# d8ahazard/AudioLab

Measured on AMD Instinct MI355X. Metric: stems*realtime-factor (44.1kHz stereo), higher is better.
Workload: dtype bf16; 1 GPU; MDX-Net UVR 4-stem (4x TFC-TDF U-Net L=11 g=48 dim_f=3072 dim_t=256 n_fft=6144), 300 s 44.1 kHz stereo in total, margin chunker, windows/launch=52; stems=4

## Files before the change

audiolab_amd/csrc/tdfnet.hip:

```cpp
#include "mma.h"
#include <alsep_gfx950_asm.h>

#include <map>
#include <type_traits>

namespace {

constexpr int kThreads = 256;

template <typename T> struct Vec16;
template <> struct Vec16<float> { static constexpr int N = 4; };
template <> struct Vec16<bf16_t> { static constexpr int N = 8; };
__device__ __forceinline__ void store_vec(float* p, const float* y) { *reinterpret_cast<float4*>(p) = make_float4(y[0], y[1], y[2], y[3]); }
__device__ __forceinline__ void store_vec(bf16_t* p, const float* y) {
    bf16x8 q;
#pragma unroll
    for (int e = 0; e < 8; ++e) q[e] = (bf16_t)y[e];
    *reinterpret_cast<bf16x8*>(p) = q;
}
__device__ __forceinline__ void load_vec(const float* p, float* x) {
    const float4 q = *reinterpret_cast<const float4*>(p);
    x[0] = q.x; x[1] = q.y; x[2] = q.z; x[3] = q.w;
}
__device__ __forceinline__ void load_vec(const bf16_t* p, float* x) {
// ... 566 lines not shown
        if (i < Cf::WINST) glds16(wsrc_next + ((size_t)i * 64 + lane) * 8, wdst_next + (size_t)i * 64 * 8);
    };

    constexpr int ST = 4 * (Cf::NPAIR + Cf::NB % 2);
    f32x4 acc[NY][3][4];
    if (nstage > 0) {
        issue_patch(0);
        weights_prep(0);
#pragma unroll
        for (int j = 0; j < 6; ++j) weights_one(j);
    }
    for (int s = 0; s < nstage; ++s) {
        const int ny = s % NY, ps = s / NY, q = ps % nq;
        const bool last = s + 1 >= nstage;
        const bool after_epilogue = ny == 0 && q == 0 && s > 0;
        if (after_epilogue) wait_vmcnt<ST>();
        else wait_vmcnt<0>();
        barrier_nodrain();
        if (!last) weights_prep(s + 1);
        {
            const bf16_t* wts = wring + (size_t)(s & 1) * Cf::WGROUPS * 8;
#pragma unroll
            for (int yy = 0; yy < NY; ++yy) {
                if (yy == ny) {
                    if (q == 0) {
#pragma unroll
                        for (int mi = 0; mi < 3; ++mi)
#pragma unroll
                            for (int ni = 0; ni < 4; ++ni) acc[yy][mi][ni] = f32x4{0.f, 0.f, 0.f, 0.f};
                    }
#pragma unroll 2
                    for (int st = 0; st < Cf::NS; ++st) {
                        const int ko = koff_of(st);
                        bf16x8 xf[4], wf[3];
#pragma unroll
                        for (int ni = 0; ni < 4; ++ni) xf[ni] = lds_frag<bf16_t>(patch + pbase[ni] + ko);
#pragma unroll
                        for (int mi = 0; mi < 3; ++mi)
                            wf[mi] = lds_frag<bf16_t>(wts + ((mi * 16 + l15) * Cf::WGRP + ((4 * st + lq) ^ wswz)) * 8);
#pragma unroll
                        for (int mi = 0; mi < 3; ++mi)
#pragma unroll
                            for (int ni = 0; ni < 4; ++ni) mma_step(acc[yy][mi][ni], wf[mi], xf[ni]);
                        if (st < 6 && !last) weights_one(st);
                    }
                }
            }
        }
        if (ny == NY - 1) {
            barrier_nodrain();
            if (!last) issue_patch(ps + 1);
            if (q == nq - 1) {
                int t0, f0; int64_t b;
                tile_coords(ps / nq, t0, f0, b);
                bf16_t* yb = Y + ((b * Th + t0 + wave) * (int64_t)Fw + f0) * Cout;
#pragma unroll
                for (int ni = 0; ni < 4; ++ni) {
                    bf16_t* yp = yb + (int64_t)(ni * 16 + l15) * Cout;
#pragma unroll
                    for (int j = 0; j < Cf::NPAIR; ++j) {
                        const int co = j * 32 + lq * 8;
                        float y[8];
#pragma unroll
                        for (int h = 0; h < 2; ++h) {
                            const int bb = 2 * j + h;
                            const f32x4 scv = *reinterpret_cast<const f32x4*>(ss + co + 4 * h);
                            const f32x4 shv = *reinterpret_cast<const f32x4*>(ss + NY * Cf::BN + co + 4 * h);
#pragma unroll
                            for (int r = 0; r < 4; ++r) y[4 * h + r] = fmaxf(fmaf(acc[bb / 3][bb % 3][ni][r], scv[r], shv[r]), 0.f);
                        }
                        store8(yp + co, y);
                    }
                    if constexpr (Cf::NB % 2 == 1) {
                        constexpr int bb = Cf::NB - 1;
                        const int co = bb * 16 + lq * 4;
                        const f32x4 scv = *reinterpret_cast<const f32x4*>(ss + co);
                        const f32x4 shv = *reinterpret_cast<const f32x4*>(ss + NY * Cf::BN + co);
                        float y[4];
#pragma unroll
                        for (int r = 0; r < 4; ++r) y[r] = fmaxf(fmaf(acc[bb / 3][bb % 3][ni][r], scv[r], shv[r]), 0.f);
                        store4(yp + co, y);
                    }
                }
            }
        }
    }
}

struct ConvMq {
    static constexpr int NY = 2, TW = 64, TH = 8, KC = 32, CG = 4, NS = 9, PW = TW + 2, PH = TH + 2;
    static constexpr int PARTS = 2, KS = 5;
    static constexpr int WG = 4 * KS, ROWS = 96, NB = 6, NPAIR = 3;
    static constexpr int PGROUPS = PH * PW * CG, PINST = (PGROUPS + 63) / 64, PJ = (PINST + 7) / 8;
    static constexpr int WGROUPS = ROWS * WG, WINST = WGROUPS / 64, WJ = (WINST + 7) / 8;
    static constexpr int PBUF = PINST * 64;
    static constexpr size_t ring_bytes = 16 * (size_t)(2 * PBUF + 2 * WGROUPS);
    static constexpr size_t lds_bytes = ring_bytes + 2 * ROWS * sizeof(float) + 1024;
    static_assert(lds_bytes <= 160 * 1024, "ConvMq: LDS budget");
    __host__ __device__ static constexpr int ksteps_of_part(int pt) { return pt == 0 ? KS : NS - KS; }
    __host__ __device__ static constexpr int wswz(int row) { return (4 - ((row >> 2) & 3)) & 3; }
    __host__ __device__ static constexpr int pswz(int pix) { return ((pix >> 2) & 1) << 1; }
};

template <int TAP, int STL>
__device__ __forceinline__ void mq_issue_reads(bf16x8 (&xf)[4], bf16x8 (&wf)[6], const bf16_t* patch, const int (&pk)[9], const bf16_t* wl) {
    typedef ConvMq Cf;
    const bf16_t* pl = patch + pk[TAP];
    lds_read_async_b128<0 * 16 * Cf::KC * 2>(xf[0], pl);
    lds_read_async_b128<1 * 16 * Cf::KC * 2>(xf[1], pl);
    lds_read_async_b128<2 * 16 * Cf::KC * 2>(xf[2], pl);
    lds_read_async_b128<3 * 16 * Cf::KC * 2>(xf[3], pl);
    lds_read_async_b128<(0 * 16 * Cf::WG * 8 + STL * 32) * 2>(wf[0], wl);
    lds_read_async_b128<(1 * 16 * Cf::WG * 8 + STL * 32) * 2>(wf[1], wl);
    lds_read_async_b128<(2 * 16 * Cf::WG * 8 + STL * 32) * 2>(wf[2], wl);
    lds_read_async_b128<(3 * 16 * Cf::WG * 8 + STL * 32) * 2>(wf[3], wl);
    lds_read_async_b128<(4 * 16 * Cf::WG * 8 + STL * 32) * 2>(wf[4], wl);
    lds_read_async_b128<(5 * 16 * Cf::WG * 8 + STL * 32) * 2>(wf[5], wl);
}
__device__ __forceinline__ void mq_mma(f32x4 (&acc)[6][4], const bf16x8 (&wf)[6], const bf16x8 (&xf)[4]) {
#pragma unroll
    for (int b = 0; b < 6; ++b)
#pragma unroll
        for (int ni = 0; ni < 4; ++ni) mma_step(acc[b][ni], wf[b], xf[ni]);
}
template <int PT, int STL, typename Dma>
__device__ __forceinline__ void mq_steps(f32x4 (&acc)[6][4], bf16x8 (&xa)[4], bf16x8 (&wa)[6], bf16x8 (&xb)[4], bf16x8 (&wb)[6],
                                         const bf16_t* patch, const int (&pk)[9], const bf16_t* wl, Dma dma) {
    constexpr int N = ConvMq::ksteps_of_part(PT), T0 = PT * ConvMq::KS;
    if constexpr (STL < N) {
        if constexpr (STL == 0) mq_issue_reads<T0, 0>(xa, wa, patch, pk, wl);
        lds_wait_n<0>();
        if constexpr (STL + 1 < N) mq_issue_reads<T0 + STL + 1, STL + 1>(xb, wb, patch, pk, wl);
        mq_mma(acc, wa, xa);
        dma(STL);
        sched_fence();
        if constexpr (STL + 1 < N) {
            lds_wait_n<0>();
            if constexpr (STL + 2 < N) mq_issue_reads<T0 + STL + 2, STL + 2>(xa, wa, patch, pk, wl);
            mq_mma(acc, wb, xb);
            dma(STL + 1);
            sched_fence();
            mq_steps<PT, STL + 2>(acc, xa, wa, xb, wb, patch, pk, wl, dma);
        }
    }
}

__global__ void __launch_bounds__(kBigThreads, 2)
conv3x3_bf16_mq_kernel(const bf16_t* __restrict__ X, bf16_t* __restrict__ Y, const bf16_t* __restrict__ Wp, const float* __restrict__ scale,
                       const float* __restrict__ shift, const bf16_t* __restrict__ zero_page, int Th, int Fw, int Cin, int Cout, int tiles_t,
                       int tiles_f, int ntiles) {
    typedef ConvMq Cf;
    bf16_t* const patch0 = reinterpret_cast<bf16_t*>(alsep_smem);
    bf16_t* const wring = patch0 + (size_t)2 * Cf::PBUF * 8;
    float* ss = reinterpret_cast<float*>(alsep_smem + Cf::ring_bytes);
    bf16_t* const scratch = reinterpret_cast<bf16_t*>(alsep_smem + Cf::lds_bytes - 1024);
    const int tid = threadIdx.x, lane = tid & 63, wave = tid >> 6;
    const int l15 = lane & 15, lq = lane >> 4;
    const int nq = Cin / Cf::KC;
    for (int i = tid; i < Cf::ROWS; i += kBigThreads) {
        ss[i] = scale[i];
        ss[Cf::ROWS + i] = shift[i];
    }
    __syncthreads();

    int pk[9];
#pragma unroll
// ... 1638 lines not shown
            for (int ni = 0; ni < P::NI; ++ni) acc[mt][ni] = f32x4{0.f, 0.f, 0.f, 0.f};
        bf16x8 xf[2][P::NI];
        static_for<P::NI>([&](auto nic) {
            constexpr int ni = decltype(nic)::value;
            lds_read_async_b128<ni * 2 * P::XREG>(xf[0][ni], xs + bk[0] / sizeof(bf16_t));
        });
        static_for<P::KS>([&](auto ksc) {
            constexpr int ks = decltype(ksc)::value, b = ks & 1;
            if constexpr (ks + 1 < P::KS) {
                static_for<P::NI>([&](auto nic) {
                    constexpr int ni = decltype(nic)::value;
                    lds_read_async_b128<ni * 2 * P::XREG>(xf[1 - b][ni], xs + bk[ks + 1] / sizeof(bf16_t));
                });
                lds_wait_n<P::NI>();
            } else {
                lds_wait_n<0>();
                if (P::C % 32 != 0) {
#pragma unroll
                    for (int ni = 0; ni < P::NI; ++ni) xf[b][ni] = klast_ok ? xf[b][ni] : bf16x8{};
                }
            }
#pragma unroll
            for (int mt = 0; mt < P::MT; ++mt)
#pragma unroll
                for (int ni = 0; ni < P::NI; ++ni) mma_step(acc[mt][ni], wf[mt][ks], xf[b][ni]);
        });
        bf16_t* sl = reinterpret_cast<bf16_t*>(sring + (size_t)(i % P::NSS) * P::s_bytes + ebase);
        const float* bnl = bn + 4 * lq;
        auto eoff = [&](int mt) {
            int t = 2 * mt + erot;
            t = t >= P::NG ? t - P::NG : t;
            return t * 8;
        };
        bf16x8 ev[2][P::NI];
        f32x4 scv[2], shv[2];
        auto eread = [&](auto mtc) {
            constexpr int mt = decltype(mtc)::value, eb = mt & 1;
            const bf16_t* p = sl + eoff(mt);
            static_for<P::NI>([&](auto nic) {
                constexpr int ni = decltype(nic)::value;
                lds_read_async_b128<ni * 32 * P::NG * 16>(ev[eb][ni], p);
            });
            lds_read_async_f32x4<0>(scv[eb], bnl + mt * 16);
            lds_read_async_f32x4<P::C2 * 4>(shv[eb], bnl + mt * 16);
        };
        eread(std::integral_constant<int, 0>{});
        static_for<P::MT>([&](auto mtc) {
            constexpr int mt = decltype(mtc)::value, b = mt & 1;
            if constexpr (mt + 1 < P::MT) {
                eread(std::integral_constant<int, mt + 1>{});
                lds_wait_n<P::NI + 2>();
            } else {
                lds_wait_n<0>();
            }
            bf16_t* p = sl + eoff(mt) + (lq & 1) * 4;
            static_for<P::NI>([&](auto nic) {
                constexpr int ni = decltype(nic)::value;
                const bf16x4 sk = (lq & 1) ? __builtin_shufflevector(ev[b][ni], ev[b][ni], 4, 5, 6, 7)
                                           : __builtin_shufflevector(ev[b][ni], ev[b][ni], 0, 1, 2, 3);
                bf16x4 q;
#pragma unroll
                for (int r = 0; r < 4; ++r) q[r] = (bf16_t)(fmaxf(fmaf(acc[mt][ni][r], scv[b][r], shv[b][r]), 0.f) * (float)sk[r]);
                lds_write_async_b64(p + ni * 32 * P::NG * 8, q);
            });
        });
    }
    barrier_nodrain();
    copy_out(nmy - 1);
}

#ifndef ALSEP_F16_TU
#include "tdfnet_f32s.h"
#endif

struct DevBuf {
    void* p = nullptr;
    size_t bytes = 0;
};

struct ConvLayer {
    DevBuf w, scale, shift;
    DevBuf w_big;
    DevBuf w_mq;
    int cin = 0, cout = 0;
    bool dma_path = false;
    int split = 0;
    unsigned* range_flag = nullptr;
};
struct GemmLayer {
    DevBuf w, bias, scale, shift;
    int M = 0, K = 0, Kp = 0, Mp = 0;
    bool has_bias = false;
    bool split = false;
    unsigned* range_flag = nullptr;
    bool dma_path = false;
    DevBuf wfrag;
    DevBuf wwide;
};
struct Block {
    std::vector<ConvLayer> tfc;
    std::vector<GemmLayer> tdf;
};

}

struct alsep_net {
    alsep_ctx* ctx = nullptr;
    alsep_net_config cfg{};
    int n = 0;
    bool split = false;
    DevBuf range_flag;
    std::vector<DevBuf> owned;
    DevBuf first_w, first_scale, first_shift, final_w, final_b, zero_page;
    std::vector<Block> enc, dec;
    Block bott;
    std::vector<GemmLayer> ds, us;
};

namespace {

typedef std::map<std::string, std::vector<float>> TensorMap;

template <typename T> T host_cast(float v);
template <> float host_cast<float>(float v) { return v; }
template <> bf16_t host_cast<bf16_t>(float v) { return (bf16_t)v; }

int upload(alsep_net* net, const void* src, size_t bytes, DevBuf* out) {
    void* d = nullptr;
    if (hipMalloc(&d, bytes ? bytes : 16) != hipSuccess) return alsep_fail(net->ctx, ALSEP_ERR_NOMEM, "hipMalloc(%zu) failed", bytes);
    out->p = d;
    out->bytes = bytes;
    net->owned.push_back(*out);
    if (bytes) ALSEP_HIP(net->ctx, hipMemcpy(d, src, bytes, hipMemcpyHostToDevice));
    return ALSEP_OK;
}

const std::vector<float>* find(const TensorMap& tm, const std::string& name, int64_t numel, alsep_ctx* ctx, bool required = true) {
    auto it = tm.find(name);
    if (it == tm.end()) {
        if (required) alsep_fail(ctx, ALSEP_ERR_ARG, "missing tensor '%s'", name.c_str());
        return nullptr;
    }
    if ((int64_t)it->second.size() != numel) {
        alsep_fail(ctx, ALSEP_ERR_ARG, "tensor '%s' has %zu elements, expected %lld", name.c_str(), it->second.size(), (long long)numel);
        return nullptr;
    }
    return &it->second;
}

template <typename T> struct ConvSel;
template <> struct ConvSel<bf16_t> { static constexpr int KC = 48, BN = 48; };
template <> struct ConvSel<float> { static constexpr int KC = 16, BN = 48; };
template <typename T> struct ConvSel16;
template <> struct ConvSel16<bf16_t> { static constexpr int KC = 16, BN = 16; };
template <> struct ConvSel16<float> { static constexpr int KC = 16, BN = 16; };

template <typename T> bool conv_uses_main(int cin, int cout) {
    return cin % ConvSel<T>::KC == 0 && cout % ConvSel<T>::BN == 0;
}

template <typename T, int KC, int BN>
std::vector<T> pack_conv3x3(const std::vector<float>& w, int cin, int cout) {
    typedef ConvCfg<T, KC, BN, 64> Cf;
    const int nq = cin / KC, nn = cout / BN;
    std::vector<T> out((size_t)nn * nq * BN * Cf::KP, host_cast<T>(0.f));
    for (int j = 0; j < nn; ++j)
        for (int q = 0; q < nq; ++q)
            for (int r = 0; r < BN; ++r)
                for (int grp = 0; grp < Cf::NG; ++grp)
                    for (int e = 0; e < Cf::G; ++e) {
                        const int tap = grp / Cf::CG, cg = grp % Cf::CG;
                        const int ci = q * KC + cg * Cf::G + e, co = j * BN + r;
                        const float v = w[(((size_t)co * cin + ci) * 3 + tap / 3) * 3 + tap % 3];
                        out[(((size_t)j * nq + q) * BN + r) * Cf::KP + grp * Cf::G + e] = host_cast<T>(v);
                    }
    return out;
}

std::vector<bf16_t> pack_conv3x3_dma(const std::vector<float>& w, int cin, int cout) {
    typedef ConvB16<64> Cf;
    const int nq = cin / Cf::KC, nn = cout / Cf::BN;
    std::vector<bf16_t> out((size_t)nn * nq * Cf::WGROUPS * 8, host_cast<bf16_t>(0.f));
    for (int j = 0; j < nn; ++j)
        for (int q = 0; q < nq; ++q)
            for (int r = 0; r < Cf::BN; ++r)
                for (int grp = 0; grp < Cf::NG; ++grp)
                    for (int e = 0; e < 8; ++e) {
                        const int tap = grp / Cf::CG, cg = grp % Cf::CG;
                        const int ci = q * Cf::KC + cg * 8 + e, co = j * Cf::BN + r;
                        const float v = w[(((size_t)co * cin + ci) * 3 + tap / 3) * 3 + tap % 3];
                        const int pg = grp ^ ((r >> 1) & 7);
                        out[((((size_t)j * nq + q) * Cf::BN + r) * Cf::WG + pg) * 8 + e] = host_cast<bf16_t>(v);
                    }
    return out;
}

template <int NY>
std::vector<bf16_t> pack_conv3x3_big(const std::vector<float>& w, int cin) {
    const int cout = 48 * NY;
    std::vector<float> wp(w.size());
    const size_t row = (size_t)cin * 9;
    for (int R = 0; R < cout; ++R) std::copy(w.begin() + ConvBig<NY>::channel_of_row(R) * row, w.begin() + (ConvBig<NY>::channel_of_row(R) + 1) * row, wp.begin() + R * row);
    return pack_conv3x3_dma(wp, cin, cout);
}

std::vector<bf16_t> pack_conv3x3_mq(const std::vector<float>& w, int cin) {
    typedef ConvMq Cf;
    const int nq = cin / Cf::KC;
    std::vector<bf16_t> out((size_t)nq * Cf::PARTS * Cf::WGROUPS * 8, host_cast<bf16_t>(0.f));
    for (int q = 0; q < nq; ++q)
        for (int pt = 0; pt < Cf::PARTS; ++pt)
            for (int R = 0; R < Cf::ROWS; ++R)
                for (int stl = 0; stl < Cf::ksteps_of_part(pt); ++stl)
                    for (int lq = 0; lq < 4; ++lq) {
                        const int tap = pt * Cf::KS + stl, co = ConvBig<2>::channel_of_row(R);
                        const size_t dst = ((((size_t)q * Cf::PARTS + pt) * Cf::ROWS + R) * Cf::WG + 4 * stl + (lq ^ Cf::wswz(R))) * 8;
                        for (int e = 0; e < 8; ++e) {
                            const int ci = q * Cf::KC + lq * 8 + e;
                            out[dst + e] = host_cast<bf16_t>(w[(((size_t)co * cin + ci) * 3 + tap / 3) * 3 + tap % 3]);
                        }
                    }
    return out;
}

template <typename T> constexpr bool is_bf16() { return false; }
template <> constexpr bool is_bf16<bf16_t>() { return true; }

template <typename T>
int make_conv(alsep_net* net, const TensorMap& tm, const std::string& p, int c, ConvLayer* L) {
    auto w = find(tm, p + ".weight", (int64_t)c * c * 9, net->ctx);
    auto sc = find(tm, p + ".scale", c, net->ctx);
    auto sh = find(tm, p + ".shift", c, net->ctx);
    if (!w || !sc || !sh) return ALSEP_ERR_ARG;
    L->cin = L->cout = c;
    int rc;
#ifndef ALSEP_F16_TU
    if (!is_bf16<T>() && net->split && (c % 48 == 0 || c % 16 == 0)) {
        L->split = c % 48 == 0 ? 24 : 16;
        L->range_flag = (unsigned*)net->range_flag.p;
        const std::vector<hs_t> pk = L->split == 24 ? pack_conv3x3_split<24, 48>(*w, c, c) : pack_conv3x3_split<16, 16>(*w, c, c);
        rc = upload(net, pk.data(), pk.size() * sizeof(hs_t), &L->w);
    } else
#endif
    if (is_bf16<T>() && c % 48 == 0) {
        L->dma_path = true;
        auto pk = pack_conv3x3_dma(*w, c, c);
        rc = upload(net, pk.data(), pk.size() * sizeof(bf16_t), &L->w);
        if (!rc && c == 48) {
            auto p0 = pack_conv3x3_big<1>(*w, c);
            rc = upload(net, p0.data(), p0.size() * sizeof(bf16_t), &L->w_big);
        }
        if (!rc && c == 96) {
            auto pq = pack_conv3x3_mq(*w, c);
            rc = upload(net, pq.data(), pq.size() * sizeof(bf16_t), &L->w_mq);
        }
        if (!rc && c == 144) {
            auto pb = pack_conv3x3_big<3>(*w, c);
            rc = upload(net, pb.data(), pb.size() * sizeof(bf16_t), &L->w_big);
        }
    } else if (conv_uses_main<T>(c, c)) {
        auto pk = pack_conv3x3<T, ConvSel<T>::KC, ConvSel<T>::BN>(*w, c, c);
        rc = upload(net, pk.data(), pk.size() * sizeof(T), &L->w);
    } else {
        auto pk = pack_conv3x3<T, ConvSel16<T>::KC, ConvSel16<T>::BN>(*w, c, c);
        rc = upload(net, pk.data(), pk.size() * sizeof(T), &L->w);
    }
    if (rc) return rc;
    if ((rc = upload(net, sc->data(), c * sizeof(float), &L->scale))) return rc;
    return upload(net, sh->data(), c * sizeof(float), &L->shift);
}

template <typename T>
int make_gemm_weights(alsep_net* net, const std::vector<float>& wmk, int M, int K, GemmLayer* L) {
    typedef GemmCfg<T> Gc;
    L->M = M; L->K = K;
#ifndef ALSEP_F16_TU
    if (!is_bf16<T>() && net->split) {
        L->split = true;
        L->range_flag = (unsigned*)net->range_flag.p;
        const std::vector<hs_t> pk = pack_gemm_split(wmk, M, K, &L->Mp, &L->Kp);
        return upload(net, pk.data(), pk.size() * sizeof(hs_t), &L->w);
    }
#endif
    L->Mp = (int)ceil_div64(M, Gc::BR) * Gc::BR;
    L->Kp = (int)ceil_div64(K, Gc::BK) * Gc::BK;
    std::vector<T> pk((size_t)L->Mp * L->Kp, host_cast<T>(0.f));
    for (int m = 0; m < M; ++m)
        for (int k = 0; k < K; ++k) pk[(size_t)m * L->Kp + k] = host_cast<T>(wmk[(size_t)m * K + k]);
    return upload(net, pk.data(), pk.size() * sizeof(T), &L->w);
}

int make_tdf_dma_weights(alsep_net* net, const std::vector<float>& wmk, int M, int K, GemmLayer* L) {
    typedef TdfB16 Tc;
    L->M = M; L->K = K;
    L->Mp = (int)ceil_div64(M, Tc::BM) * Tc::BM;
    L->Kp = (int)ceil_div64(K, Tc::BK) * Tc::BK;
    L->dma_path = true;
    std::vector<bf16_t> pk((size_t)L->Mp * L->Kp, host_cast<bf16_t>(0.f));
    for (int m = 0; m < M; ++m)
        for (int kt = 0; kt < L->Kp / Tc::BK; ++kt)
            for (int g = 0; g < 8; ++g) {
                const int ks = g >> 2, lq = g & 3, pg = g ^ ((m >> 1) & 7);
                for (int e = 0; e < 8; ++e) {
                    const int k = kt * Tc::BK + ks * 32 + (e < 4 ? 4 * lq + e : 16 + 4 * lq + (e - 4));
                    if (k < K) pk[(size_t)m * L->Kp + kt * Tc::BK + pg * 8 + e] = host_cast<bf16_t>(wmk[(size_t)m * K + k]);
                }
            }
    return upload(net, pk.data(), pk.size() * sizeof(bf16_t), &L->w);
}

int make_tdf_wide_weights(alsep_net* net, const std::vector<float>& wmk, int M, int K, GemmLayer* L) {
    const int KT = (int)ceil_div64(K, 64);
    std::vector<bf16_t> pk((size_t)(M / 48) * KT * 6 * 512, host_cast<bf16_t>(0.f));
    for (int rb = 0; rb < M / 48; ++rb)
        for (int kt = 0; kt < KT; ++kt)
            for (int ks = 0; ks < 2; ++ks)
                for (int mi = 0; mi < 3; ++mi)
                    for (int l = 0; l < 64; ++l)
                        for (int e = 0; e < 8; ++e) {
                            const int lq = l >> 4, m = rb * 48 + mi * 16 + (l & 15);
                            const int k = kt * 64 + ks * 32 + (e < 4 ? 4 * lq + e : 16 + 4 * lq + (e - 4));
                            if (k < K)
                                pk[((((size_t)rb * KT + kt) * 2 + ks) * 3 + mi) * 512 + l * 8 + e] =
                                    host_cast<bf16_t>(wmk[(size_t)m * K + k]);
                        }
    return upload(net, pk.data(), pk.size() * sizeof(bf16_t), &L->wwide);
}

int make_frag_weights(alsep_net* net, const std::vector<float>& wmk, int M, int K, DevBuf* out) {
    const int MT = (M + 15) / 16, KS = (K + 31) / 32;
    std::vector<bf16_t> pk((size_t)MT * KS * 64 * 8, host_cast<bf16_t>(0.f));
    for (int mt = 0; mt < MT; ++mt)
        for (int ks = 0; ks < KS; ++ks)
            for (int l = 0; l < 64; ++l)
                for (int e = 0; e < 8; ++e) {
                    const int m = mt * 16 + (l & 15), k = ks * 32 + (l >> 4) * 8 + e;
                    if (m < M && k < K) pk[(((size_t)mt * KS + ks) * 64 + l) * 8 + e] = host_cast<bf16_t>(wmk[(size_t)m * K + k]);
                }
    return upload(net, pk.data(), pk.size() * sizeof(bf16_t), out);
}

template <typename T>
// ... 125 lines not shown
    return v;
}

template <int TW>
int launch_conv_dma(alsep_ctx* ctx, const ConvLayer& L, const bf16_t* X, bf16_t* Y, const bf16_t* zero_page, int64_t B,
                    int Th, int Fw) {
    typedef ConvB16<TW> Cf;
    const int tiles_t = (int)ceil_div64(Th, Cf::TH), tiles_f = (int)ceil_div64(Fw, TW);
    const int64_t ntiles = B * tiles_t * tiles_f;
    if (ntiles > 0x7fffffff) return alsep_fail(ctx, ALSEP_ERR_ARG, "conv3x3: too many tiles");
    ALSEP_HIP(ctx, hipFuncSetAttribute((const void*)conv3x3_bf16_kernel<TW>, hipFuncAttributeMaxDynamicSharedMemorySize,
                                       (int)Cf::lds_bytes));
    ProfScope prof(ctx, TW == 64 ? ALSEP_PROF_CONV3X3 : ALSEP_PROF_CONV3X3_SMALL);
    prof.work(18.0 * (double)L.cin * L.cout * B * Th * Fw, (double)sizeof(*X) * B * Th * Fw * (L.cin + L.cout));
    const int nyc = L.cout / Cf::BN;
    const int ny_fastest = conv_ny_fastest() && ntiles % 8 == 0 && nyc > 1 && ntiles * nyc <= 0x7fffffff;
    hipLaunchKernelGGL((conv3x3_bf16_kernel<TW>), ny_fastest ? dim3((unsigned)(ntiles * nyc)) : dim3((unsigned)ntiles, nyc),
                       dim3(kThreads), Cf::lds_bytes,
                       ctx->stream, X, Y, (const bf16_t*)L.w.p, (const float*)L.scale.p, (const float*)L.shift.p, zero_page,
                       Th, Fw, L.cin, L.cout, tiles_t, tiles_f, (int)ntiles,  0,  0, ny_fastest);
    note_launch(ctx, TW == 64 ? "conv3x3_bf16_kernel<64>" : "conv3x3_bf16_kernel<small>");
    ALSEP_LAUNCH_CHECK(ctx, "conv3x3_bf16_kernel");
    return ALSEP_OK;
}

template <int NQ, int RING_ = 3, int OCC = 1, int TW_ = 64>
int launch_conv_regw(alsep_ctx* ctx, const ConvLayer& L, const bf16_t* X, bf16_t* Y, const bf16_t* zero_page, int64_t B,
                     int Th, int Fw) {
    typedef ConvRW<NQ, RING_, TW_> Cf;
    const int tiles_t = Th / Cf::TH, tiles_f = Fw / Cf::TW;
    const int64_t ntiles = B * tiles_t * tiles_f;
    if (ntiles > 0x7fffffff) return alsep_fail(ctx, ALSEP_ERR_ARG, "conv3x3: too many tiles");
    ALSEP_HIP(ctx, hipFuncSetAttribute((const void*)conv3x3_bf16_regw_kernel<NQ, RING_, OCC, TW_>,
                                       hipFuncAttributeMaxDynamicSharedMemorySize, (int)Cf::lds_bytes));
    const int ny = L.cout / Cf::BN;
    int gx = OCC * 256 / ny;
    if (gx > ntiles) gx = (int)ntiles;
    ProfScope prof(ctx, ALSEP_PROF_CONV3X3_REGW);
    prof.work(18.0 * (double)L.cin * L.cout * B * Th * Fw, (double)sizeof(*X) * B * Th * Fw * (L.cin + L.cout));
    hipLaunchKernelGGL((conv3x3_bf16_regw_kernel<NQ, RING_, OCC, TW_>), dim3((unsigned)gx, ny), dim3(kThreads), Cf::lds_bytes, ctx->stream, X, Y,
                       (const bf16_t*)L.w.p, (const float*)L.scale.p, (const float*)L.shift.p, zero_page, Th, Fw, L.cin,
                       L.cout, tiles_t, tiles_f, (int)ntiles);
    ALSEP_LAUNCH_CHECK(ctx, "conv3x3_bf16_regw_kernel");
    return ALSEP_OK;
}

template <typename Cf, typename Kern>
int launch_conv_persist(alsep_ctx* ctx, Kern kern, const ConvLayer& L, const DevBuf& wimg, int prof_class, const char* name, const bf16_t* X,
                        bf16_t* Y, const bf16_t* zero_page, int64_t B, int Th, int Fw) {
    const int tiles_t = Th / Cf::TH, tiles_f = Fw / Cf::TW;
    const int64_t ntiles = B * tiles_t * tiles_f;
    if (ntiles > 0x7fffffff) return alsep_fail(ctx, ALSEP_ERR_ARG, "conv3x3: too many tiles");
    ALSEP_HIP(ctx, hipFuncSetAttribute((const void*)kern, hipFuncAttributeMaxDynamicSharedMemorySize, (int)Cf::lds_bytes));
    const int gx = ntiles < 256 ? (int)ntiles : 256;
    ProfScope prof(ctx, prof_class);
    prof.work(18.0 * (double)L.cin * L.cout * B * Th * Fw, (double)sizeof(*X) * B * Th * Fw * (L.cin + L.cout));
    hipLaunchKernelGGL(kern, dim3((unsigned)gx), dim3(kBigThreads), Cf::lds_bytes, ctx->stream, X, Y, (const bf16_t*)wimg.p,
                       (const float*)L.scale.p, (const float*)L.shift.p, zero_page, Th, Fw, L.cin, L.cout, tiles_t, tiles_f, (int)ntiles);
    ALSEP_LAUNCH_CHECK(ctx, name);
    return ALSEP_OK;
}

int launch_conv_big3(alsep_ctx* ctx, const ConvLayer& L, const bf16_t* X, bf16_t* Y, const bf16_t* zero_page, int64_t B, int Th, int Fw) {
    if (!L.w_big.p) return alsep_fail(ctx, ALSEP_ERR_STATE, "conv3x3: no big-tile weight image for this layer");
    if (int rc = launch_conv_persist<ConvBig<3>>(ctx, conv3x3_bf16_big_kernel<3>, L, L.w_big, ALSEP_PROF_CONV3X3_BIG3, "conv3x3_bf16_big_kernel",
                                                 X, Y, zero_page, B, Th, Fw))
        return rc;
    note_launch(ctx, "conv3x3_bf16_big_kernel<3>");
    return ALSEP_OK;
}

int launch_conv_mq(alsep_ctx* ctx, const ConvLayer& L, const bf16_t* X, bf16_t* Y, const bf16_t* zero_page, int64_t B, int Th, int Fw) {
    if (!L.w_mq.p || L.cout != ConvMq::ROWS || L.cin % ConvMq::KC) return alsep_fail(ctx, ALSEP_ERR_STATE, "conv3x3: no mq weight image for this layer");
    return launch_conv_persist<ConvMq>(ctx, conv3x3_bf16_mq_kernel, L, L.w_mq, ALSEP_PROF_CONV3X3_BIG, "conv3x3_bf16_mq_kernel", X, Y, zero_page,
                                       B, Th, Fw);
}

int launch_conv_m0(alsep_ctx* ctx, const ConvLayer& L, const bf16_t* X, bf16_t* Y, const bf16_t* zero_page, int64_t B, int Th, int Fw) {
    if (!L.w_big.p || L.cout != ConvM0::ROWS || L.cin != ConvM0::KC) return alsep_fail(ctx, ALSEP_ERR_STATE, "conv3x3: no m0 weight image for this layer");
    return launch_conv_persist<ConvM0>(ctx, conv3x3_bf16_m0_kernel, L, L.w_big, ALSEP_PROF_CONV3X3_REGW, "conv3x3_bf16_m0_kernel", X, Y, zero_page,
                                       B, Th, Fw);
}

int conv_m0_enabled() {
    static const int v = env_int("ALSEP_CONV_M0", 1);
    return v;
}
int conv_regw_enabled() {
    static const int v = env_int("ALSEP_CONV_REGW", 1);
    return v;
}
int conv_big_enabled() {
    static const int v = env_int("ALSEP_CONV_BIG", 1);
    return v;
}
int conv_mq_enabled() {
    static const int v = env_int("ALSEP_CONV_MQ", 1);
    return v;
}
int conv_big3_enabled() {
    static const int v = env_int("ALSEP_CONV_BIG3", 1);
    return v;
}

int run_conv_dma(alsep_ctx* ctx, const ConvLayer& L, const bf16_t* X, bf16_t* Y, const bf16_t* zp, int64_t B, int Th, int Fw) {
    if (conv_m0_enabled() && L.cin == 48 && L.cout == 48 && Th % 8 == 0 && Fw % 48 == 0 &&
        (conv_m0_enabled() >= 2 || B * (Th / 8) * (Fw / 48) >= 256))
        return launch_conv_m0(ctx, L, X, Y, zp, B, Th, Fw);
    if (conv_regw_enabled() && Th % 4 == 0 && Fw % 64 == 0 && L.cin == L.cout) {
        if (L.cin == 48 && conv_regw_enabled() == 3) return launch_conv_regw<1>(ctx, L, X, Y, zp, B, Th, Fw);
        if (L.cin == 48) return launch_conv_regw<1, 3, 2, 32>(ctx, L, X, Y, zp, B, Th, Fw);
        if (L.cin == 96 && conv_regw_enabled() >= 2) return launch_conv_regw<2>(ctx, L, X, Y, zp, B, Th, Fw);
    }
    if (conv_big_enabled() && Th % 8 == 0 && Fw % 64 == 0 && L.cin == L.cout &&
        (conv_big_enabled() >= 2 || B * (Th / 8) * (Fw / 64) >= 96)) {
        if (L.cout == 96 && conv_mq_enabled()) return launch_conv_mq(ctx, L, X, Y, zp, B, Th, Fw);
        if (L.cout == 144 && conv_big3_enabled()) return launch_conv_big3(ctx, L, X, Y, zp, B, Th, Fw);
    }
    if (Fw >= 64 && Fw % 64 == 0) return launch_conv_dma<64>(ctx, L, X, Y, zp, B, Th, Fw);
    if (Fw >= 32) return launch_conv_dma<32>(ctx, L, X, Y, zp, B, Th, Fw);
    return launch_conv_dma<16>(ctx, L, X, Y, zp, B, Th, Fw);
}
int run_conv_dma(alsep_ctx* ctx, const ConvLayer&, const float*, float*, const float*, int64_t, int, int) {
    return alsep_fail(ctx, ALSEP_ERR_STATE, "LDS-DMA conv path is bf16 only");
}

#ifndef ALSEP_F16_TU
template <int KC, int BN, int TW>
int launch_conv_split(alsep_ctx* ctx, const ConvLayer& L, const float* X, float* Y, int64_t B, int Th, int Fw) {
    typedef ConvSCfg<KC, BN, TW> Cf;
    const int tiles_t = (int)ceil_div64(Th, Cf::TH), tiles_f = (int)ceil_div64(Fw, TW);
    const int64_t ntiles = B * tiles_t * tiles_f;
    const int nyc = L.cout / BN;
    if (ntiles * nyc > 0x7fffffff) return alsep_fail(ctx, ALSEP_ERR_ARG, "conv3x3: too many tiles");
    ALSEP_HIP(ctx, hipFuncSetAttribute((const void*)conv3x3_f32s_kernel<KC, BN, TW>, hipFuncAttributeMaxDynamicSharedMemorySize,
                                       (int)Cf::lds_bytes));
    ProfScope prof(ctx, TW >= 32 ? ALSEP_PROF_CONV3X3 : ALSEP_PROF_CONV3X3_SMALL);
    prof.work(18.0 * (double)L.cin * L.cout * B * Th * Fw, 4.0 * B * Th * Fw * (L.cin + L.cout));
    const int nyf = (ntiles % 8 == 0 && nyc > 1) ? 1 : 0;
    const dim3 grid = nyf ? dim3((unsigned)(ntiles * nyc)) : dim3((unsigned)ntiles, nyc);
    hipLaunchKernelGGL((conv3x3_f32s_kernel<KC, BN, TW>), grid, dim3(kThreads), Cf::lds_bytes, ctx->stream, X, Y,
                       (const hs_t*)L.w.p, (const float*)L.scale.p, (const float*)L.shift.p, Th, Fw, L.cin, L.cout, tiles_t, tiles_f,
                       (int)ntiles, nyf, L.range_flag);
    ALSEP_LAUNCH_CHECK(ctx, "conv3x3_f32s_kernel");
    return ALSEP_OK;
}
template <int KC, int BN>
int run_conv_split_tw(alsep_ctx* ctx, const ConvLayer& L, const float* X, float* Y, int64_t B, int Th, int Fw) {
    if (Fw >= 32) return launch_conv_split<KC, BN, 32>(ctx, L, X, Y, B, Th, Fw);
    return launch_conv_split<KC, BN, 16>(ctx, L, X, Y, B, Th, Fw);
}
int run_conv_split(alsep_ctx* ctx, const ConvLayer& L, const float* X, float* Y, int64_t B, int Th, int Fw) {
    return L.split == 24 ? run_conv_split_tw<24, 48>(ctx, L, X, Y, B, Th, Fw) : run_conv_split_tw<16, 16>(ctx, L, X, Y, B, Th, Fw);
}
int run_conv_split(alsep_ctx* ctx, const ConvLayer&, const bf16_t*, bf16_t*, int64_t, int, int) {
    return alsep_fail(ctx, ALSEP_ERR_STATE, "split contraction is a float32 mode");
}
#endif

template <typename T>
int run_conv(alsep_ctx* ctx, const ConvLayer& L, const T* X, T* Y, int64_t B, int Th, int Fw, const void* zero_page) {
#ifndef ALSEP_F16_TU
    if (L.split) return run_conv_split(ctx, L, X, Y, B, Th, Fw);
#endif
    if (L.dma_path) return run_conv_dma(ctx, L, X, Y, (const T*)zero_page, B, Th, Fw);
    if (conv_uses_main<T>(L.cin, L.cout)) return run_conv_tw<T, ConvSel<T>::KC, ConvSel<T>::BN>(ctx, L, X, Y, B, Th, Fw);
    return run_conv_tw<T, ConvSel16<T>::KC, ConvSel16<T>::BN>(ctx, L, X, Y, B, Th, Fw);
}

int pix_stream_enabled() {
    static const int v = env_int("ALSEP_PIX_STREAM", 1);
    return v;
}
enum { kPixPipeDs96 = 1, kPixPipeDs144 = 2, kPixPipeUs192 = 4, kPixPipeUs144 = 8 };
constexpr int kPixPipeRouted = kPixPipeDs96 | kPixPipeDs144 | kPixPipeUs192 | kPixPipeUs144;
bool pix_pipe_routed(int kind) {
    static const int v = env_int("ALSEP_PIX_PIPE", 1);
    return v >= 2 || (v == 1 && (kPixPipeRouted & kind));
}
unsigned pix_pipe_grid(alsep_ctx* ctx, int64_t ntile) {
    static const int cap = env_int("ALSEP_PIX_PIPE_GRID", 0);
    int64_t grid = device_cu_count(ctx);
    if (cap > 0 && cap < grid) grid = cap;
    return (unsigned)std::min<int64_t>(grid, ntile);
}
template <int C_, int PX_, int D_>
hipError_t launch_ds_pipe(alsep_ctx* ctx, const GemmLayer& L, const bf16_t* X, bf16_t* Y, int64_t ncols, int Tp, int Fp) {
    typedef DsPipeCfg<C_, PX_, D_> P;
    const hipError_t e = hipFuncSetAttribute((const void*)ds_pipe_kernel<C_, PX_, D_>, hipFuncAttributeMaxDynamicSharedMemorySize, (int)P::lds_bytes);
    if (e != hipSuccess) return e;
    hipLaunchKernelGGL((ds_pipe_kernel<C_, PX_, D_>), dim3(pix_pipe_grid(ctx, ncols / P::PX)), dim3(kThreads), P::lds_bytes, ctx->stream, X, Y,
                       (const bf16_t*)L.wfrag.p, (const float*)L.scale.p, (const float*)L.shift.p, ncols, Tp, Fp);
    return hipSuccess;
}
template <int CIN, int C2_, int NI_, int D_>
hipError_t launch_us_pipe(alsep_ctx* ctx, const GemmLayer& L, const bf16_t* X, bf16_t* Y, const bf16_t* skip, int64_t ncols, int Tp, int Fp) {
    typedef UsPipeCfg<CIN, C2_, NI_, D_> P;
    const hipError_t e = hipFuncSetAttribute((const void*)us_pipe_kernel<CIN, C2_, NI_, D_>, hipFuncAttributeMaxDynamicSharedMemorySize, (int)P::lds_bytes);
    if (e != hipSuccess) return e;
    hipLaunchKernelGGL((us_pipe_kernel<CIN, C2_, NI_, D_>), dim3(pix_pipe_grid(ctx, ncols / P::PX)), dim3(kThreads), P::lds_bytes, ctx->stream, X, Y,
// ... 528 lines not shown
```

Before: 6171 stems*x_realtime.

## Add persistent grouped-channel conv3x3 kernel for 192-channel layers

Adds a persistent conv3x3 kernel that splits 192/240/288-channel outputs into two groups of 2–3 48-channel blocks. It streams double-buffered weights through LDS and prefetches input patches, overlapping each group's epilogue stores with the next item's loads. By default it routes only 192-channel layers, replacing the generic DMA conv path for them. The trade-off is extra weight images, more LDS use and more complex scheduling, and input patches are loaded twice per tile, once per group.

```diff
diff --git a/audiolab_amd/csrc/tdfnet.hip b/audiolab_amd/csrc/tdfnet.hip
--- a/audiolab_amd/csrc/tdfnet.hip
+++ b/audiolab_amd/csrc/tdfnet.hip
@@ -672,6 +672,215 @@
                         store4(yp + co, y);
                     }
                 }
+            }
+        }
+    }
+}
+
+struct ConvGrp {
+    typedef ConvBig<3> Geo;
+    static constexpr int NYMAX = 3, MAXC = 288;
+    static constexpr size_t lds_bytes = Geo::ring_bytes + 2 * MAXC * sizeof(float);
+    static_assert(lds_bytes <= 160 * 1024, "ConvGrp: LDS budget");
+    __host__ __device__ static constexpr bool serves(int c) { return c == 192 || c == 240 || c == 288; }
+    __host__ __device__ static constexpr int first_group(int nyt) { return (nyt + 1) / 2; }
+    __host__ __device__ static inline void item_of(int i, int ntiles, int& tile, int& g) {
+        const int nblk = (ntiles / 8) * 16;
+        if (i < nblk) {
+            tile = (i >> 4) * 8 + (i & 7);
+            g = ((i >> 3) ^ (i >> 8)) & 1;
+        } else {
+            tile = (ntiles / 8) * 8 + ((i - nblk) >> 1);
+            g = (i - nblk) & 1;
+        }
+    }
+};
+
+__global__ void __launch_bounds__(kBigThreads, 2)
+conv3x3_bf16_grp_kernel(const bf16_t* __restrict__ X, bf16_t* __restrict__ Y, const bf16_t* __restrict__ Wp,
+                        const float* __restrict__ scale, const float* __restrict__ shift,
+                        const bf16_t* __restrict__ zero_page, int Th, int Fw, int Cin, int Cout, int tiles_t,
+                        int tiles_f, int ntiles) {
+    typedef ConvGrp::Geo Cf;
+    bf16_t* patch = reinterpret_cast<bf16_t*>(alsep_smem);
+    bf16_t* wring = patch + (size_t)Cf::PGROUPS * 8;
+    float* ss = reinterpret_cast<float*>(alsep_smem + Cf::ring_bytes);
+    const int tid = threadIdx.x, lane = tid & 63, wave = tid >> 6;
+    const int l15 = lane & 15, lq = lane >> 4;
+    const int nq = Cin / Cf::KC, nyt = Cout / Cf::BN, n0 = ConvGrp::first_group(nyt);
+    const int wswz = l15 >> 1;
+    for (int i = tid; i < Cout; i += kBigThreads) {
+        ss[i] = scale[i];
+        ss[Cout + i] = shift[i];
+    }
+    __syncthreads();
+
+    int pbase[4];
+#pragma unroll
+    for (int ni = 0; ni < 4; ++ni) pbase[ni] = (wave * Cf::PW + ni * 16 + l15) * Cf::KC;
+    auto koff_of = [&](int s) {
+        const int grp = 4 * s + lq;
+        const int gc = grp < Cf::NG ? grp : Cf::NG - 1;
+        const int tap = gc / Cf::CG, cg = gc % Cf::CG;
+        return ((tap / 3) * Cf::PW + (tap % 3)) * Cf::KC + cg * 8;
+    };
+    const int nitems = 2 * ntiles;
+    const int my_items = (nitems - (int)blockIdx.x + (int)gridDim.x - 1) / (int)gridDim.x;
+
+    auto item_coords = [&](int k, int& t0, int& f0, int64_t& b, int& g) {
+        int tile;
+        ConvGrp::item_of((int)blockIdx.x + k * (int)gridDim.x, ntiles, tile, g);
+        const int tf = tile % tiles_f;  tile /= tiles_f;
+        const int tt = tile % tiles_t;
+        b = tile / tiles_t;
+        t0 = tt * Cf::TH;
+        f0 = tf * Cf::TW;
+    };
+    constexpr int PJ = (Cf::PINST + 7) / 8;
+    int prel[PJ];
+    unsigned pflags = 0;
+    bool plast_ok = true;
+#pragma unroll
+    for (int j = 0; j < PJ; ++j) {
+        const int gidx = (wave + 8 * j) * 64 + lane;
+        const int gi = gidx < Cf::PGROUPS ? gidx : Cf::PGROUPS - 1;
+        const int pix = gi / Cf::CG, g = gi % Cf::CG;
+        const int dt = pix / Cf::PW - 1, df = pix % Cf::PW - 1;
+        prel[j] = (dt * Fw + df) * Cin + g * 8;
+        pflags |= (unsigned)((dt < 0) | ((dt >= Cf::TH) << 1) | ((df < 0) << 2) | ((df >= Cf::TW) << 3)) << (4 * j);
+        if (j == PJ - 1) plast_ok = gidx < Cf::PGROUPS;
+    }
+    auto issue_patch = [&](int k, int q) {
+        int t0, f0, g; int64_t b;
+        item_coords(k, t0, f0, b, g);
+        const bf16_t* xb = X + ((b * Th + t0) * (int64_t)Fw + f0) * Cin + q * Cf::KC;
+        const unsigned border = (unsigned)(t0 == 0) | ((unsigned)(t0 + Cf::TH >= Th) << 1) | ((unsigned)(f0 == 0) << 2) |
+                                ((unsigned)(f0 + Cf::TW >= Fw) << 3);
+#pragma unroll
+        for (int j = 0; j < PJ; ++j) {
+            const int i = wave + 8 * j;
+            if (j < PJ - 1 || i < Cf::PINST) {
+                const bool out = (pflags & (border << (4 * j))) != 0;
+                const bf16_t* src = out ? zero_page : xb + prel[j];
+                if (j < PJ - 1 || plast_ok) glds16(src, patch + (size_t)i * 64 * 8);
+            }
+        }
+    };
+    const bf16_t* wsrc_next = Wp;
+    bf16_t* wdst_next = wring;
+    auto weights_prep = [&](int ny, int q, int slot) {
+        wsrc_next = Wp + ((int64_t)ny * nq + q) * (Cf::WGROUPS * 8);
+        wdst_next = wring + (size_t)slot * Cf::WGROUPS * 8;
+    };
+    auto weights_one = [&](int j) {
+        const int i = wave + 8 * j;
+        if (i < Cf::WINST) glds16(wsrc_next + ((size_t)i * 64 + lane) * 8, wdst_next + (size_t)i * 64 * 8);
+    };
+    f32x4 acc[ConvGrp::NYMAX][3][4];
+    auto epilogue = [&](auto gc, int t0, int f0, int64_t b, int c0) {
+        typedef ConvBig<decltype(gc)::value> Cg;
+        bf16_t* yb = Y + ((b * Th + t0 + wave) * (int64_t)Fw + f0) * Cout + c0;
+        const float* sc = ss + c0;
+        const float* sh = ss + Cout + c0;
+#pragma unroll
+        for (int ni = 0; ni < 4; ++ni) {
+            bf16_t* yp = yb + (int64_t)(ni * 16 + l15) * Cout;
+#pragma unroll
+            for (int j = 0; j < Cg::NPAIR; ++j) {
+                const int co = j * 32 + lq * 8;
+                float y[8];
+#pragma unroll
+                for (int h = 0; h < 2; ++h) {
+                    const int bb = 2 * j + h;
+                    const f32x4 scv = *reinterpret_cast<const f32x4*>(sc + co + 4 * h);
+                    const f32x4 shv = *reinterpret_cast<const f32x4*>(sh + co + 4 * h);
+#pragma unroll
+                    for (int r = 0; r < 4; ++r) y[4 * h + r] = fmaxf(fmaf(acc[bb / 3][bb % 3][ni][r], scv[r], shv[r]), 0.f);
+                }
+                store8(yp + co, y);
+            }
+            if constexpr (Cg::NB % 2 == 1) {
+                constexpr int bb = Cg::NB - 1;
+                const int co = bb * 16 + lq * 4;
+                const f32x4 scv = *reinterpret_cast<const f32x4*>(sc + co);
+                const f32x4 shv = *reinterpret_cast<const f32x4*>(sh + co);
+                float y[4];
+#pragma unroll
+                for (int r = 0; r < 4; ++r) y[r] = fmaxf(fmaf(acc[bb / 3][bb % 3][ni][r], scv[r], shv[r]), 0.f);
+                store4(yp + co, y);
+            }
+        }
+    };
+
+    constexpr int ST2 = 4 * (ConvBig<2>::NPAIR + ConvBig<2>::NB % 2), ST3 = 4 * (ConvBig<3>::NPAIR + ConvBig<3>::NB % 2);
+    int slot = 0, stored = 0;
+    if (my_items > 0) {
+        int t0, f0, g; int64_t b;
+        item_coords(0, t0, f0, b, g);
+        issue_patch(0, 0);
+        weights_prep(g ? n0 : 0, 0, 0);
+#pragma unroll
+        for (int j = 0; j < 6; ++j) weights_one(j);
+    }
+    for (int k = 0; k < my_items; ++k) {
+        int t0, f0, g; int64_t b;
+        item_coords(k, t0, f0, b, g);
+        const int ny0 = g ? n0 : 0, gny = g ? nyt - n0 : n0;
+        const bool last_item = k + 1 >= my_items;
+        int next_ny0 = 0;
+        if (!last_item) {
+            int t1, f1, g1; int64_t b1;
+            item_coords(k + 1, t1, f1, b1, g1);
+            next_ny0 = g1 ? n0 : 0;
+        }
+        for (int q = 0; q < nq; ++q) {
+            const bool last_chunk = q + 1 >= nq;
+#pragma unroll
+            for (int yy = 0; yy < ConvGrp::NYMAX; ++yy) {
+                if (yy < 2 || gny == 3) {
+                    const bool last_block = yy + 1 >= gny;
+                    const bool last = last_item && last_chunk && last_block;
+                    if (yy == 0 && q == 0 && stored == 3) wait_vmcnt<ST3>();
+                    else if (yy == 0 && q == 0 && stored == 2) wait_vmcnt<ST2>();
+                    else wait_vmcnt<0>();
+                    barrier_nodrain();
+                    if (!last) {
+                        if (!last_block) weights_prep(ny0 + yy + 1, q, slot ^ 1);
+                        else if (!last_chunk) weights_prep(ny0, q + 1, slot ^ 1);
+                        else weights_prep(next_ny0, 0, slot ^ 1);
+                    }
+                    const bf16_t* wts = wring + (size_t)slot * Cf::WGROUPS * 8;
+                    if (q == 0) {
+#pragma unroll
+                        for (int mi = 0; mi < 3; ++mi)
+#pragma unroll
+                            for (int ni = 0; ni < 4; ++ni) acc[yy][mi][ni] = f32x4{0.f, 0.f, 0.f, 0.f};
+                    }
+#pragma unroll 2
+                    for (int st = 0; st < Cf::NS; ++st) {
+                        const int ko = koff_of(st);
+                        bf16x8 xf[4], wf[3];
+#pragma unroll
+                        for (int ni = 0; ni < 4; ++ni) xf[ni] = lds_frag<bf16_t>(patch + pbase[ni] + ko);
+#pragma unroll
+                        for (int mi = 0; mi < 3; ++mi)
+                            wf[mi] = lds_frag<bf16_t>(wts + ((mi * 16 + l15) * Cf::WGRP + ((4 * st + lq) ^ wswz)) * 8);
+#pragma unroll
+                        for (int mi = 0; mi < 3; ++mi)
+#pragma unroll
+                            for (int ni = 0; ni < 4; ++ni) mma_step(acc[yy][mi][ni], wf[mi], xf[ni]);
+                        if (st < 6 && !last) weights_one(st);
+                    }
+                    slot ^= 1;
+                }
+            }
+            barrier_nodrain();
+            if (!last_chunk) issue_patch(k, q + 1);
+            else if (!last_item) issue_patch(k + 1, 0);
+            if (last_chunk) {
+                if (gny == 3) epilogue(std::integral_constant<int, 3>(), t0, f0, b, ny0 * Cf::BN);
+                else epilogue(std::integral_constant<int, 2>(), t0, f0, b, ny0 * Cf::BN);
+                stored = gny;
             }
         }
     }
@@ -2476,6 +2685,7 @@
     DevBuf w, scale, shift;
     DevBuf w_big;
     DevBuf w_mq;
+    DevBuf w_grp;
     int cin = 0, cout = 0;
     bool dma_path = false;
     int split = 0;
@@ -2596,6 +2806,27 @@
     const size_t row = (size_t)cin * 9;
     for (int R = 0; R < cout; ++R) std::copy(w.begin() + ConvBig<NY>::channel_of_row(R) * row, w.begin() + (ConvBig<NY>::channel_of_row(R) + 1) * row, wp.begin() + R * row);
     return pack_conv3x3_dma(wp, cin, cout);
+}
+
+template <int NY>
+void append_conv3x3_group(std::vector<bf16_t>& out, const std::vector<float>& w, int cin, int c0) {
+    const size_t row = (size_t)cin * 9;
+    std::vector<float> wg((size_t)48 * NY * row);
+    for (int R = 0; R < 48 * NY; ++R) {
+        const size_t src = (size_t)(c0 + ConvBig<NY>::channel_of_row(R)) * row;
+        std::copy(w.begin() + src, w.begin() + src + row, wg.begin() + R * row);
+    }
+    const std::vector<bf16_t> img = pack_conv3x3_dma(wg, cin, 48 * NY);
+    out.insert(out.end(), img.begin(), img.end());
+}
+std::vector<bf16_t> pack_conv3x3_grp(const std::vector<float>& w, int c) {
+    const int nyt = c / 48, n0 = ConvGrp::first_group(nyt);
+    std::vector<bf16_t> out;
+    if (n0 == 3) append_conv3x3_group<3>(out, w, c, 0);
+    else append_conv3x3_group<2>(out, w, c, 0);
+    if (nyt - n0 == 3) append_conv3x3_group<3>(out, w, c, 48 * n0);
+    else append_conv3x3_group<2>(out, w, c, 48 * n0);
+    return out;
 }
 
 std::vector<bf16_t> pack_conv3x3_mq(const std::vector<float>& w, int cin) {
@@ -2652,6 +2883,10 @@
             auto pb = pack_conv3x3_big<3>(*w, c);
             rc = upload(net, pb.data(), pb.size() * sizeof(bf16_t), &L->w_big);
         }
+        if (!rc && ConvGrp::serves(c)) {
+            auto pg = pack_conv3x3_grp(*w, c);
+            rc = upload(net, pg.data(), pg.size() * sizeof(bf16_t), &L->w_grp);
+        }
     } else if (conv_uses_main<T>(c, c)) {
         auto pk = pack_conv3x3<T, ConvSel<T>::KC, ConvSel<T>::BN>(*w, c, c);
         rc = upload(net, pk.data(), pk.size() * sizeof(T), &L->w);
@@ -2943,6 +3178,28 @@
                                        B, Th, Fw);
 }
 
+int launch_conv_grp(alsep_ctx* ctx, const ConvLayer& L, const bf16_t* X, bf16_t* Y, const bf16_t* zero_page, int64_t B, int Th, int Fw) {
+    typedef ConvGrp::Geo Cf;
+    static const int cap = env_int("ALSEP_CONV_GROUPS_GRID", 0);
+    if (!L.w_grp.p || !ConvGrp::serves(L.cout) || L.cin != L.cout) return alsep_fail(ctx, ALSEP_ERR_STATE, "conv3x3: no group weight images for this layer");
+    const int tiles_t = Th / Cf::TH, tiles_f = Fw / Cf::TW;
+    const int64_t ntiles = B * tiles_t * tiles_f;
+    if (ntiles > 0x3fffffff) return alsep_fail(ctx, ALSEP_ERR_ARG, "conv3x3: too many tiles");
+    ALSEP_HIP(ctx, hipFuncSetAttribute((const void*)conv3x3_bf16_grp_kernel, hipFuncAttributeMaxDynamicSharedMemorySize, (int)ConvGrp::lds_bytes));
+    int64_t grid = device_cu_count(ctx);
+    if (cap > 0 && cap < grid) grid = cap;
+    if (2 * ntiles < grid) grid = 2 * ntiles;
+    ProfScope prof(ctx, ALSEP_PROF_CONV3X3);
+    prof.work(18.0 * (double)L.cin * L.cout * B * Th * Fw, (double)sizeof(*X) * B * Th * Fw * (L.cin + L.cout));
+    hipLaunchKernelGGL(conv3x3_bf16_grp_kernel, dim3((unsigned)grid), dim3(kBigThreads), ConvGrp::lds_bytes, ctx->stream, X, Y,
+                       (const bf16_t*)L.w_grp.p, (const float*)L.scale.p, (const float*)L.shift.p, zero_page, Th, Fw, L.cin, L.cout, tiles_t,
+                       tiles_f, (int)ntiles);
+    note_launch(ctx, "conv3x3_bf16_kernel<64>");
+    note_launch(ctx, "conv3x3_bf16_kernel");
+    ALSEP_LAUNCH_CHECK(ctx, "conv3x3_bf16_grp_kernel");
+    return ALSEP_OK;
+}
+
 int conv_m0_enabled() {
     static const int v = env_int("ALSEP_CONV_M0", 1);
     return v;
@@ -2962,6 +3219,14 @@
 int conv_big3_enabled() {
     static const int v = env_int("ALSEP_CONV_BIG3", 1);
     return v;
+}
+
+enum { kConvGroups192 = 1, kConvGroups240 = 2, kConvGroups288 = 4 };
+constexpr int kConvGroupsRouted = kConvGroups192;
+bool conv_groups_routed(int c) {
+    static const int v = env_int("ALSEP_CONV_GROUPS", 1);
+    const int kind = c == 192 ? kConvGroups192 : c == 240 ? kConvGroups240 : kConvGroups288;
+    return v >= 2 || (v == 1 && (kConvGroupsRouted & kind));
 }
 
 int run_conv_dma(alsep_ctx* ctx, const ConvLayer& L, const bf16_t* X, bf16_t* Y, const bf16_t* zp, int64_t B, int Th, int Fw) {
@@ -2977,6 +3242,7 @@
         (conv_big_enabled() >= 2 || B * (Th / 8) * (Fw / 64) >= 96)) {
         if (L.cout == 96 && conv_mq_enabled()) return launch_conv_mq(ctx, L, X, Y, zp, B, Th, Fw);
         if (L.cout == 144 && conv_big3_enabled()) return launch_conv_big3(ctx, L, X, Y, zp, B, Th, Fw);
+        if (ConvGrp::serves(L.cout) && conv_groups_routed(L.cout)) return launch_conv_grp(ctx, L, X, Y, zp, B, Th, Fw);
     }
     if (Fw >= 64 && Fw % 64 == 0) return launch_conv_dma<64>(ctx, L, X, Y, zp, B, Th, Fw);
     if (Fw >= 32) return launch_conv_dma<32>(ctx, L, X, Y, zp, B, Th, Fw);
```

After: 6188 stems*x_realtime, median of 3. No clear change (+0.3%).
